# zeroQiaoba/MERTools

Measured on NVIDIA H100. Metric: clips/sec tri-modal feature-extract + fusion-train step, higher is better.
Workload: dtype f16 operands (ViT / HuBERT / BERT layers, ViT attention) / tf32 (audio + text attention, patch embed) / f16 (HuBERT conv1-2) / bf16x3 (HuBERT conv3-6, feature projection) tensor-core products, fp32 accumulate; fp32 elsewhere

## Files before the change

mertools_b200/_lib.py:

```python
from __future__ import annotations

import ctypes as C
import os

_HERE = os.path.dirname(os.path.abspath(__file__))
LIB_PATH = os.path.join(_HERE, "lib", "libmer_b200.so")

MER_EPI_GELU = 1
MER_EPI_ROUND_TF32 = 2
MER_EPI_SPLIT_BF16 = 4
MER_GEMM_TF32 = 0
MER_GEMM_BF16X3 = 1
MER_GEMM_F16 = 2
MER_EPI_OUT_F16 = 16
MER_LN_OUT_F16 = 8
MER_ATT_QKV_F16 = 32
MER_LN_ROUND_TF32 = 1
MER_LN_ACC_INIT = 2
MER_LN_ACC_ADD = 4


class MerError(RuntimeError):
    pass


class MerGemmEpilogue(C.Structure):
    _fields_ = [
        ("bias", C.c_void_p), ("res", C.c_void_p), ("out", C.c_void_p),
        ("out_bstride", C.c_longlong), ("out_row0", C.c_longlong),
        ("res_bstride", C.c_longlong), ("res_row0", C.c_longlong),
        ("ld_out", C.c_int), ("ld_res", C.c_int), ("flags", C.c_int), ("split_off", C.c_int),
        ("vt", C.c_void_p), ("vt_ld", C.c_longlong), ("vt_col0", C.c_int),
    ]


class MerGemmDesc(C.Structure):
    _fields_ = [
        ("A", C.c_void_p), ("W", C.c_void_p),
        ("rows_per_batch", C.c_int), ("a_rows_dim", C.c_int), ("batches", C.c_int),
        ("N", C.c_int), ("K_inner", C.c_int), ("taps", C.c_int), ("P", C.c_int),
        ("a_phase_stride", C.c_longlong), ("a_row_stride", C.c_longlong),
        ("a_batch_stride", C.c_longlong), ("force_block_n", C.c_int), ("mode", C.c_int),
        ("cluster", C.c_int), ("a_row0", C.c_int), ("a_cols", C.c_int), ("a_col_group", C.c_int),
        ("ep", MerGemmEpilogue),
    ]


_lib = None


def lib() -> C.CDLL:
    global _lib
    if _lib is None:
        if not os.path.exists(LIB_PATH):
            raise MerError(
                f"{LIB_PATH} not found: run `python -c 'import __graft_entry__ as g; g.build()'` "
                "(no CPU fallback exists for the mertools_b200 hot path)")
        _lib = C.CDLL(LIB_PATH)
        _lib.mer_last_error.restype = C.c_char_p
        _declare(_lib)
    return _lib


def _declare(l):
    vp, i32, i64, f32 = C.c_void_p, C.c_int, C.c_longlong, C.c_float
    sig = {
        "mer_abi_version": [],
        "mer_check_device": [],
        "mer_gemm": [C.POINTER(MerGemmDesc), vp],
        "mer_layernorm": [vp, vp, vp, vp, vp, vp, i64, i32, f32, i32, vp],
        "mer_round_tf32": [vp, i64, vp],
        "mer_split_bf16": [vp, vp, i64, i32, vp],
        "mer_attention": [vp, vp, i64, vp, vp, i32, i64, i32, i32, i32, vp],
    }
    for name, args in sig.items():
        fn = getattr(l, name)
        fn.argtypes = args
        fn.restype = C.c_int


def declare(name, args):
    fn = getattr(lib(), name)
    fn.argtypes = args
    fn.restype = C.c_int
    return fn


def check(rc: int):
    if rc != 0:
        raise MerError(f"libmer_b200 error {rc}: {lib().mer_last_error().decode(errors='replace')}")


def ptr(t):
    if t is None:
        return None
    return C.c_void_p(t.data_ptr())


def stream_ptr():
    import torch
    return C.c_void_p(torch.cuda.current_stream().cuda_stream)


def gemm(A, W, out, *, bias=None, res=None, gelu=False, round_out=False, split_out=False,
         mode=MER_GEMM_TF32, rows_per_batch=None, batches=1, a_rows_dim=None, K_inner=None, taps=1, P=1,
         a_phase_stride=0, a_row_stride=None, a_batch_stride=0,
         out_bstride=0, out_row0=0, res_bstride=0, res_row0=0,
         ld_out=None, ld_res=None, force_block_n=0, cluster=0, vt=None, vt_col0=0, gelu_libm=False,
         f16_out=False, a_row0=0, a_cols=0, a_col_group=0):
    N, K = W.shape
    d = MerGemmDesc()
    d.A, d.W = A.data_ptr(), W.data_ptr()
    d.taps, d.P = taps, P
    d.K_inner = K_inner if K_inner is not None else K // taps
    assert d.K_inner * taps == K
    d.rows_per_batch = rows_per_batch if rows_per_batch is not None else A.shape[0]
    d.a_rows_dim = a_rows_dim if a_rows_dim is not None else d.rows_per_batch
    d.batches = batches
    d.N = N
    d.a_phase_stride = a_phase_stride if P > 1 else d.K_inner
    d.a_row_stride = a_row_stride if a_row_stride is not None else K
    d.a_batch_stride = a_batch_stride if batches > 1 else d.a_row_stride * d.a_rows_dim
    d.force_block_n = force_block_n
    d.mode = mode
    d.cluster = cluster
    d.a_row0, d.a_cols, d.a_col_group = a_row0, a_cols, a_col_group
    d.ep.bias = bias.data_ptr() if bias is not None else None
    d.ep.res = res.data_ptr() if res is not None else None
    d.ep.out = out.data_ptr()
    d.ep.out_bstride, d.ep.out_row0 = out_bstride, out_row0
    d.ep.res_bstride, d.ep.res_row0 = res_bstride, res_row0
    d.ep.ld_out = ld_out if ld_out is not None else N
    d.ep.ld_res = ld_res if ld_res is not None else N
    d.ep.flags = ((MER_EPI_GELU if gelu else 0) | (MER_EPI_ROUND_TF32 if round_out else 0)
                  | (MER_EPI_SPLIT_BF16 if split_out else 0) | (8 if gelu_libm else 0)
                  | (MER_EPI_OUT_F16 if f16_out else 0))
    d.ep.split_off = N
    if vt is not None:
        d.ep.vt, d.ep.vt_ld, d.ep.vt_col0 = vt.data_ptr(), vt.shape[1], vt_col0
    check(lib().mer_gemm(C.byref(d), stream_ptr()))
    return out


gemm_tf32 = gemm


def layernorm(x, gamma, beta, y, *, eps, y_split=None, acc=None, flags=0):
    rows = x.numel() // x.shape[-1]
    check(lib().mer_layernorm(ptr(x), ptr(gamma), ptr(beta), ptr(y), ptr(y_split), ptr(acc), rows,
                              x.shape[-1], eps, flags, stream_ptr()))
    return y


def split_bf16(x):
    import torch
    x = x.contiguous()
    out = torch.empty_like(x)
    check(lib().mer_split_bf16(ptr(x), ptr(out), x.numel() // x.shape[-1], x.shape[-1], stream_ptr()))
    return out


def unsplit_bf16(xs):
    import torch
    K = xs.shape[-1]
    b = xs.contiguous().view(torch.bfloat16).view(*xs.shape[:-1], K // 32, 2, 32).float()
    return (b[..., 0, :] + b[..., 1, :]).reshape(*xs.shape[:-1], K)


def round_tf32_(x):
    check(lib().mer_round_tf32(ptr(x), x.numel(), stream_ptr()))
    return x


def attention(qkv, ctx, cu_seqlens, max_seqlen, heads, round_out=False, vt=None, f16_out=False, split_out=False):
    import torch
    if qkv.dtype == torch.float16:
        assert vt is not None and vt.dtype == torch.float16
        if ctx.dtype == torch.float16:
            out_fl = MER_EPI_OUT_F16
        else:
            assert ctx.dtype == torch.float32
            out_fl = MER_EPI_SPLIT_BF16 if split_out else (MER_EPI_ROUND_TF32 if round_out else 0)
        check(lib().mer_attention(ptr(qkv), ptr(vt), vt.shape[1], ptr(ctx), ptr(cu_seqlens),
                                  cu_seqlens.numel() - 1, qkv.shape[0], max_seqlen, heads,
                                  out_fl | MER_ATT_QKV_F16, stream_ptr()))
        return ctx
    check(lib().mer_attention(ptr(qkv), ptr(vt), vt.shape[1] if vt is not None else 0, ptr(ctx),
                              ptr(cu_seqlens), cu_seqlens.numel() - 1, qkv.shape[0], max_seqlen, heads,
                              MER_EPI_OUT_F16 if f16_out else (MER_EPI_ROUND_TF32 if round_out else 0),
                              stream_ptr()))
    return ctx
```

mertools_b200/csrc/gemm.cu:

```cuda
#include <stdlib.h>

#include "mer_common.cuh"
#include "mer_kernels.h"

namespace {

using namespace mer;

constexpr int BLOCK_M = 128;
constexpr int BLOCK_K = 32;
constexpr int CONSUMERS = 2;
constexpr int NUM_THREADS = 128 * (1 + CONSUMERS);

template <int BLOCK_N, int MODE>
struct GemmCfg {
  static constexpr bool kSplit = MODE == MER_GEMM_BF16X3;
  static constexpr bool kF16 = MODE == MER_GEMM_F16;
  static constexpr int kBlockK = kF16 ? 64 : BLOCK_K;
  static constexpr int kRowBytes = 128;
  static constexpr int kKind = kSplit ? 1 : (kF16 ? 0 : 2);
  static constexpr int kABytes = BLOCK_M * kRowBytes;
  static constexpr int kBBytes = BLOCK_N * kRowBytes;
  static constexpr int kStageBytes = kABytes + kBBytes;
  static constexpr int kStages = BLOCK_N == 256 ? 4 : 6;
  static constexpr int kBarBytes = 256;
  static constexpr int kSmemBytes = kStages * kStageBytes + kBarBytes + 1024;
  static_assert(kSmemBytes <= 227 * 1024, "shared memory budget");
};

constexpr int EPI_GELU_PACKED = 1 << 16;

template <int GELU>
__device__ __forceinline__ float epi_act(float v) {
  if (GELU == 1) return gelu_erf_fast(v);
  if (GELU == 2) return gelu_erf(v);
  if (GELU == 3) return quick_gelu_fast(v);
  return v;
}
template <int GELU>
__device__ __forceinline__ void epi_act2(float a, float b, float& ga, float& gb) {
  if (GELU == 5) {
    gelu_erf_fast2(a, b, ga, gb);
  } else {
    ga = epi_act<GELU>(a);
    gb = epi_act<GELU>(b);
  }
}

template <int NH, int GELU, int OUT, bool RES>
__device__ __forceinline__ void epi_tile(float (&acc)[NH][64], const MerGemmEpilogue& ep, int n_base, int m_base,
                                         int rows_per_batch, long long out_row_b, long long res_row_b, int wg_row0) {
  constexpr bool kVt = GELU == 0 && !RES;
  const int lane = threadIdx.x & 31, w = (threadIdx.x >> 5) & 3;
  const int g = lane >> 2, t = lane & 3;
#pragma unroll
  for (int i = 0; i < 2; ++i) {
    const int m = m_base + wg_row0 + 16 * w + g + 8 * i;
    if (m >= rows_per_batch) continue;
    const long long orow = out_row_b + m;
    const float* rrow = RES ? ep.res + (res_row_b + m) * (long long)ep.ld_res : nullptr;
#pragma unroll
    for (int hh = 0; hh < NH; ++hh) {
#pragma unroll
      for (int j = 0; j < 16; ++j) {
        const int n = n_base + 128 * hh + 8 * j + 2 * t;
        float v0 = acc[hh][4 * j + 2 * i], v1 = acc[hh][4 * j + 2 * i + 1];
        if (ep.bias) {
          const float2 q = __ldg(reinterpret_cast<const float2*>(ep.bias + n));
          v0 += q.x;
          v1 += q.y;
        }
        if (kVt && ep.vt != nullptr && n >= ep.vt_col0) {
          const long long vo = (long long)(n - ep.vt_col0) * ep.vt_ld + orow;
          if (OUT == 3) {
            uint16_t* vt16 = reinterpret_cast<uint16_t*>(ep.vt) + vo;
            const uint32_t p = pack_f16x2(v0, v1);
            vt16[0] = (uint16_t)(p & 0xffffu);
            vt16[ep.vt_ld] = (uint16_t)(p >> 16);
          } else {
            if (OUT == 1) {
              v0 = round_tf32(v0);
              v1 = round_tf32(v1);
            }
            ep.vt[vo] = v0;
            ep.vt[vo + ep.vt_ld] = v1;
          }
          continue;
        }
        epi_act2<GELU>(v0, v1, v0, v1);
        if (RES) {
          const float2 r = __ldg(reinterpret_cast<const float2*>(rrow + n));
          v0 += r.x;
          v1 += r.y;
        }
        if (GELU == 4) {
          v0 = fmaxf(v0, 0.f);
          v1 = fmaxf(v1, 0.f);
        }
        if (OUT == 3) {
          *reinterpret_cast<uint32_t*>(reinterpret_cast<uint16_t*>(ep.out) + orow * ep.ld_out + n) = pack_f16x2(v0, v1);
        } else if (OUT == 2) {
          store_split2(ep.out + orow * ep.ld_out, n, v0, v1);
        } else {
          if (OUT == 1) {
            v0 = round_tf32(v0);
            v1 = round_tf32(v1);
          }
          *reinterpret_cast<float2*>(ep.out + orow * ep.ld_out + n) = make_float2(v0, v1);
        }
      }
    }
  }
}

template <int BLOCK_N, int MODE>
__global__ void __launch_bounds__(NUM_THREADS, 1)
gemm_kernel(const __grid_constant__ CUtensorMap tmap_a,
            const __grid_constant__ CUtensorMap tmap_b, const MerGemmEpilogue ep,
            int rows_per_batch, int batches, int N, int K, int K_inner, int P, int a_row0, int a_col_group) {
  using Cfg = GemmCfg<BLOCK_N, MODE>;
  constexpr int NH = BLOCK_N / 128;
  extern __shared__ uint8_t smem_raw[];
  uint8_t* smem = smem_raw + ((1024u - (smem_u32(smem_raw) & 1023u)) & 1023u);
  uint8_t* smem_a = smem;
  uint8_t* smem_b = smem + Cfg::kStages * Cfg::kABytes;
  uint64_t* bars = reinterpret_cast<uint64_t*>(smem + Cfg::kStages * Cfg::kStageBytes);
  uint64_t* full_bar = bars;
  uint64_t* empty_bar = bars + Cfg::kStages;

  const int wg = threadIdx.x >> 7;
  const int warp = threadIdx.x >> 5;
  const int lane = threadIdx.x & 31;

  const int m_tiles = (rows_per_batch + BLOCK_M - 1) / BLOCK_M;
  const int n_tiles = N / BLOCK_N;
  const int num_kb = K / Cfg::kBlockK;
  const int num_tiles = batches * m_tiles * n_tiles;

  if (threadIdx.x == 0) {
    tma_prefetch_desc(&tmap_a);
    tma_prefetch_desc(&tmap_b);
    for (int i = 0; i < Cfg::kStages; ++i) {
      mbar_init(&full_bar[i], 1);
      mbar_init(&empty_bar[i], 4 * CONSUMERS);
    }
    fence_mbar_init();
  }
  __syncthreads();

  if (wg == 0) {
    asm volatile("setmaxnreg.dec.sync.aligned.u32 40;\n" ::: "memory");
    if (warp != 0) return;
    int stage = 0;
    uint32_t phase = 0;
    constexpr int kEl = Cfg::kSplit ? 2 : 1;
    for (int t = blockIdx.x; t < num_tiles; t += gridDim.x) {
      const int n_blk = t % n_tiles;
      const int mb = t / n_tiles;
      const int b = mb / m_tiles;
      const int mt = mb % m_tiles;
      int c0 = 0, tap_phase = 0, tap_row = 0;
      const int c_win = a_col_group > 0 ? ((n_blk * BLOCK_N) / a_col_group) * a_col_group : 0;
      const int row_base = mt * BLOCK_M + a_row0;
      for (int kb = 0; kb < num_kb; ++kb) {
        mbar_wait_nocall(&empty_bar[stage], phase ^ 1);
        if (elect_one()) {
          mbar_expect_tx(&full_bar[stage], Cfg::kStageBytes);
          tma_load_4d(smem_a + stage * Cfg::kABytes, &tmap_a, &full_bar[stage], (c_win + c0) * kEl, tap_phase,
                      row_base + tap_row, b);
          tma_load_2d(smem_b + stage * Cfg::kBBytes, &tmap_b, &full_bar[stage], kb * Cfg::kBlockK * kEl,
                      n_blk * BLOCK_N);
        }
        __syncwarp();
        c0 += Cfg::kBlockK;
        if (c0 == K_inner) {
          c0 = 0;
          if (++tap_phase == P) {
            tap_phase = 0;
            ++tap_row;
          }
        }
        if (++stage == Cfg::kStages) {
          stage = 0;
          phase ^= 1;
        }
      }
    }
    return;
  }

  asm volatile("setmaxnreg.inc.sync.aligned.u32 232;\n" ::: "memory");
  const int wg_row0 = (wg - 1) * 64;
  const uint64_t desc_a0 = wgmma_desc_sw128(smem_u32(smem_a + wg_row0 * Cfg::kRowBytes));
  const uint64_t desc_b0 = wgmma_desc_sw128(smem_u32(smem_b));
  const int gelu_kind = (ep.flags & MER_EPI_RELU) ? 4 : (ep.flags & MER_EPI_QUICK_GELU) ? 3
                        : (ep.flags & MER_EPI_GELU)
                            ? ((ep.flags & MER_EPI_GELU_LIBM) ? 2 : ((ep.flags & EPI_GELU_PACKED) ? 5 : 1)) : 0;
  const int out_kind = (ep.flags & MER_EPI_OUT_F16) ? 3 : (ep.flags & MER_EPI_SPLIT_BF16) ? 2 :
                       ((ep.flags & MER_EPI_ROUND_TF32) ? 1 : 0);
  const int kind = gelu_kind * 4 + out_kind;
  int stage = 0;
  uint32_t phase = 0;
  float acc[NH][64];
  for (int t = blockIdx.x; t < num_tiles; t += gridDim.x) {
    const int n_blk = t % n_tiles;
    const int mb = t / n_tiles;
    const int b = mb / m_tiles;
    const int mt = mb % m_tiles;
    int prev_stage = -1;
    for (int kb = 0; kb < num_kb; ++kb) {
      mbar_wait_nocall(&full_bar[stage], phase);
      const uint64_t da = desc_a0 + (uint64_t)(stage * (Cfg::kABytes >> 4));
      const uint64_t db = desc_b0 + (uint64_t)(stage * (Cfg::kBBytes >> 4));
      constexpr uint64_t kHalfB = (128 * Cfg::kRowBytes) >> 4;
      wgmma_fence();
#pragma unroll
      for (int k = 0; k < (Cfg::kSplit ? 2 : 4); ++k) {
#pragma unroll
        for (int hh = 0; hh < NH; ++hh) {
          const uint64_t dbh = db + hh * kHalfB;
          if (!Cfg::kSplit) {
            wgmma_m64n128<Cfg::kKind>(acc[hh], da + 2 * k, dbh + 2 * k, (kb | k) != 0);
          } else {
            wgmma_m64n128<1>(acc[hh], da + 2 * k, dbh + 2 * k, (kb | k) != 0);
            wgmma_m64n128<1>(acc[hh], da + 4 + 2 * k, dbh + 2 * k, 1);
            wgmma_m64n128<1>(acc[hh], da + 2 * k, dbh + 4 + 2 * k, 1);
          }
        }
      }
      wgmma_commit();
      wgmma_wait<1>();
      if (prev_stage >= 0 && lane == 0) mbar_arrive(&empty_bar[prev_stage]);
      prev_stage = stage;
      if (++stage == Cfg::kStages) {
        stage = 0;
        phase ^= 1;
      }
    }
    wgmma_wait<0>();
#pragma unroll
    for (int hh = 0; hh < NH; ++hh)
#pragma unroll
      for (int r = 0; r < 64; ++r) wgmma_fence_operand(acc[hh][r]);
    if (lane == 0) mbar_arrive(&empty_bar[prev_stage]);

    const int n_base = n_blk * BLOCK_N;
    const int m_base = mt * BLOCK_M;
    const long long out_row_b = (long long)b * ep.out_bstride + ep.out_row0;
    const long long res_row_b = (long long)b * ep.res_bstride + ep.res_row0;
#define MER_EPI(G, O, R) epi_tile<NH, G, O, R>(acc, ep, n_base, m_base, rows_per_batch, out_row_b, res_row_b, wg_row0)
    if (ep.res != nullptr) {
      if (gelu_kind == 4) MER_EPI(4, 0, true);
      else if (gelu_kind != 0) MER_EPI(1, 0, true);
      else if (out_kind == 1) MER_EPI(0, 1, true);
      else MER_EPI(0, 0, true);
    } else {
      switch (kind) {
        case 0: MER_EPI(0, 0, false); break;
        case 1: MER_EPI(0, 1, false); break;
        case 2: MER_EPI(0, 2, false); break;
        case 3: MER_EPI(0, 3, false); break;
        case 4: MER_EPI(1, 0, false); break;
        case 5: MER_EPI(1, 1, false); break;
        case 6: MER_EPI(1, 2, false); break;
        case 7: MER_EPI(1, 3, false); break;
        case 8: MER_EPI(2, 0, false); break;
        case 9: MER_EPI(2, 1, false); break;
        case 10: MER_EPI(2, 2, false); break;
        case 11: MER_EPI(2, 3, false); break;
        case 13: MER_EPI(3, 1, false); break;
        case 15: MER_EPI(3, 3, false); break;
        case 16: MER_EPI(4, 0, false); break;
        case 22: MER_EPI(5, 2, false); break;
        case 23: MER_EPI(5, 3, false); break;
        default: MER_EPI(3, 0, false); break;
      }
    }
#undef MER_EPI
  }
}

long long g_variant_launches[8] = {};

template <int BLOCK_N, int MODE>
int launch_gemm(const MerGemmDesc* g, cudaStream_t stream) {
  using Cfg = GemmCfg<BLOCK_N, MODE>;
  ++g_variant_launches[(MODE & 3) | (BLOCK_N == 256 ? 4 : 0)];
  CUtensorMap ta, tb;
  const CUtensorMapDataType dt = Cfg::kSplit ? CU_TENSOR_MAP_DATA_TYPE_BFLOAT16
                                 : Cfg::kF16 ? CU_TENSOR_MAP_DATA_TYPE_FLOAT16
                                             : CU_TENSOR_MAP_DATA_TYPE_FLOAT32;
  const CUtensorMapSwizzle sw = CU_TENSOR_MAP_SWIZZLE_128B;
  const uint64_t mult = Cfg::kSplit ? 2 : 1;
  const uint64_t sbytes = Cfg::kF16 ? 2 : 4;
  {
    const uint64_t dims[4] = {(uint64_t)(g->a_cols > 0 ? g->a_cols : g->K_inner) * mult, (uint64_t)g->P,
                              (uint64_t)g->a_rows_dim, (uint64_t)g->batches};
    const uint64_t strides[3] = {(uint64_t)g->a_phase_stride * sbytes,
                                 (uint64_t)g->a_row_stride * sbytes,
                                 (uint64_t)g->a_batch_stride * sbytes};
    const uint32_t box[4] = {(uint32_t)(Cfg::kBlockK * mult), 1, BLOCK_M, 1};
    if (int rc = mer_make_tmap(&ta, dt, 4, g->A, dims, strides, box, sw)) return rc;
  }
  {
    const int K = g->K_inner * g->taps;
    const uint64_t dims[2] = {(uint64_t)K * mult, (uint64_t)g->N};
    const uint64_t strides[1] = {(uint64_t)K * sbytes};
    const uint32_t box[2] = {(uint32_t)(Cfg::kBlockK * mult), BLOCK_N};
    if (int rc = mer_make_tmap(&tb, dt, 2, g->W, dims, strides, box, sw)) return rc;
  }
  static MerPerDevice attr_set;
  if (attr_set.needs_setup()) {
    MER_CUDA_CHECK(cudaFuncSetAttribute(gemm_kernel<BLOCK_N, MODE>, cudaFuncAttributeMaxDynamicSharedMemorySize,
                                        Cfg::kSmemBytes));
    attr_set.mark();
  }
  const int m_tiles = (g->rows_per_batch + BLOCK_M - 1) / BLOCK_M;
  const long long tiles = (long long)g->batches * m_tiles * (g->N / BLOCK_N);
  MER_REQUIRE(tiles < (1ll << 31), "mer_gemm: %lld tiles", tiles);
  int grid = mer_num_sms();
  if (tiles < grid) grid = (int)tiles;
  const int klass = (MODE == MER_GEMM_F16 && (long long)g->rows_per_batch * g->batches < (1ll << 17)) ? MER_PROF_F16_SMALL
                                                                                                        : MODE;
  const int prof = mer_prof_begin(klass, 2.0 * (double)g->rows_per_batch * g->batches * g->N *
                                             (double)(g->K_inner * g->taps), stream);
  MerGemmEpilogue ep = g->ep;
  {
    const bool plain_gelu = (ep.flags & MER_EPI_GELU) && !(ep.flags & MER_EPI_GELU_LIBM) && !ep.res;
    if (plain_gelu && (ep.flags & (MER_EPI_OUT_F16 | MER_EPI_SPLIT_BF16))) {
      const char* e = getenv("MER_GELU_PACKED");
      if (e && atoi(e) == 1) ep.flags |= EPI_GELU_PACKED;
    }
  }
  gemm_kernel<BLOCK_N, MODE><<<grid, NUM_THREADS, Cfg::kSmemBytes, stream>>>(
      ta, tb, ep, g->rows_per_batch, g->batches, g->N, g->K_inner * g->taps, g->K_inner, g->P, g->a_row0,
      g->a_col_group);
  MER_CUDA_CHECK(cudaGetLastError());
  mer_count_launches(1);
  mer_prof_end(prof, stream);
  return 0;
}

}

extern "C" long long mer_gemm_variant_launches(int block_n, int mode, int cluster, int twosm) {
  if ((block_n != 128 && block_n != 256) || mode < 0 || mode > 2 || cluster < 1 || cluster > 2) return -1;
  if (cluster != 1 || twosm) return 0;
  return g_variant_launches[(mode & 3) | (block_n == 256 ? 4 : 0)];
}

int mer_gemm_launch(const MerGemmDesc* g, cudaStream_t stream) {
  MER_REQUIRE(g && g->A && g->W && g->ep.out, "mer_gemm: null operand");
  MER_REQUIRE(g->mode == MER_GEMM_TF32 || g->mode == MER_GEMM_BF16X3 || g->mode == MER_GEMM_F16,
              "mer_gemm: unknown mode %d", g->mode);
  const int kstep = g->mode == MER_GEMM_F16 ? 64 : BLOCK_K;
  const int salign = g->mode == MER_GEMM_F16 ? 8 : 4;

  MER_REQUIRE(g->K_inner > 0 && g->K_inner % kstep == 0 && g->taps > 0 && g->P > 0,
              "mer_gemm: K_inner=%d must be a positive multiple of %d (taps=%d P=%d)",
              g->K_inner, kstep, g->taps, g->P);
  MER_REQUIRE(g->a_rows_dim >= g->rows_per_batch, "mer_gemm: a_rows_dim < rows_per_batch");
  MER_REQUIRE(g->N > 0 && g->N % 128 == 0, "mer_gemm: N=%d must be a multiple of 128", g->N);
  MER_REQUIRE(g->rows_per_batch > 0 && g->batches > 0, "mer_gemm: empty problem");
  MER_REQUIRE(g->a_row_stride % salign == 0 && g->a_batch_stride % salign == 0 &&
                  g->a_phase_stride % salign == 0,
              "mer_gemm: A strides must be multiples of 16 bytes");
  MER_REQUIRE(!((g->ep.flags & MER_EPI_OUT_F16) &&
                ((g->ep.flags & (MER_EPI_SPLIT_BF16 | MER_EPI_ROUND_TF32)) || g->ep.res)),
              "mer_gemm: an fp16 output excludes the other output formats and a residual");
  MER_REQUIRE(g->ep.ld_out % 4 == 0 && (g->ep.res == nullptr || g->ep.ld_res % 4 == 0),
              "mer_gemm: out/res leading dims must be multiples of 4 floats");
  MER_REQUIRE(!((g->ep.flags & MER_EPI_SPLIT_BF16) && (g->ep.res || g->ep.vt)),
              "mer_gemm: a bf16-split output cannot be combined with a residual or the transposed side output");
  MER_REQUIRE(!(g->ep.res && g->ep.vt), "mer_gemm: a residual cannot be combined with the transposed side output");
  MER_REQUIRE(!(g->ep.res && (g->ep.flags & MER_EPI_GELU) &&
                (g->ep.flags & (MER_EPI_ROUND_TF32 | MER_EPI_GELU_LIBM))),
              "mer_gemm: residual + GELU is available with the polynomial GELU and a plain fp32 output");
  MER_REQUIRE(!((g->ep.flags & MER_EPI_QUICK_GELU) &&
                ((g->ep.flags & (MER_EPI_GELU | MER_EPI_SPLIT_BF16)) || g->ep.res || g->ep.vt)),
              "mer_gemm: quick-GELU comes alone (fp32, tf32 or fp16 output; no residual / split / V^T)");
  MER_REQUIRE(!((g->ep.flags & MER_EPI_RELU) &&
                ((g->ep.flags & (MER_EPI_GELU | MER_EPI_QUICK_GELU | MER_EPI_SPLIT_BF16 | MER_EPI_ROUND_TF32 |
                                 MER_EPI_OUT_F16)) || g->ep.vt)),
              "mer_gemm: ReLU goes with a plain fp32 output (optionally + residual)");
  MER_REQUIRE(g->a_col_group == 0 || g->force_block_n == 128 || g->force_block_n == 256,
              "mer_gemm: a_col_group needs force_block_n (the weights are built for one block width)");
  MER_REQUIRE(!(g->ep.vt && (g->ep.flags & MER_EPI_GELU)), "mer_gemm: GELU + transposed side output is not supported");
  const int m_tiles = (g->rows_per_batch + BLOCK_M - 1) / BLOCK_M;
  const long long tiles256 = (g->N % 256 == 0) ? (long long)g->batches * m_tiles * (g->N / 256) : 0;
  const bool wide = (tiles256 >= mer_num_sms() && g->force_block_n != 128) ||
                    (g->force_block_n == 256 && tiles256 > 0);
  if (g->mode == MER_GEMM_F16)
    return wide ? launch_gemm<256, MER_GEMM_F16>(g, stream) : launch_gemm<128, MER_GEMM_F16>(g, stream);
  if (g->mode == MER_GEMM_BF16X3)
    return wide ? launch_gemm<256, MER_GEMM_BF16X3>(g, stream) : launch_gemm<128, MER_GEMM_BF16X3>(g, stream);
  return wide ? launch_gemm<256, MER_GEMM_TF32>(g, stream) : launch_gemm<128, MER_GEMM_TF32>(g, stream);
}
```

mertools_b200/csrc/mer_common.cuh:

```cuda
#pragma once

#include <cuda.h>
#include <cuda_runtime.h>
#include <stdint.h>
#include <stdio.h>
#include <string.h>

void mer_set_error(const char* fmt, ...);

#define MER_CUDA_CHECK(expr)                                                              \
  do {                                                                                    \
    cudaError_t _e = (expr);                                                              \
    if (_e != cudaSuccess) {                                                              \
      mer_set_error("%s:%d: %s -> %s", __FILE__, __LINE__, #expr, cudaGetErrorString(_e)); \
      return 1;                                                                           \
    }                                                                                     \
  } while (0)

#define MER_REQUIRE(cond, ...)      \
  do {                              \
    if (!(cond)) {                  \
      mer_set_error(__VA_ARGS__);   \
      return 2;                     \
    }                               \
  } while (0)

int mer_make_tmap(CUtensorMap* out, CUtensorMapDataType dtype, int rank, const void* base,
                  const uint64_t* dims, const uint64_t* strides_bytes, const uint32_t* box,
                  CUtensorMapSwizzle swizzle);

int mer_num_sms();
void mer_count_launches(int n);

#ifdef __CUDACC__

#ifndef MER_SPIN_LIMIT
#define MER_SPIN_LIMIT (1u << 27)
#endif

namespace mer {

__device__ __forceinline__ uint32_t smem_u32(const void* p) {
  return static_cast<uint32_t>(__cvta_generic_to_shared(p));
}

__device__ __forceinline__ bool elect_one() {
  uint32_t pred = 0;
  asm volatile(
      "{\n\t"
      ".reg .pred P;\n\t"
      "elect.sync _|P, 0xffffffff;\n\t"
      "selp.b32 %0, 1, 0, P;\n\t"
      "}\n"
      : "=r"(pred));
  return pred != 0;
}

__device__ __forceinline__ void mbar_init(uint64_t* bar, uint32_t count) {
  asm volatile("mbarrier.init.shared::cta.b64 [%0], %1;" ::"r"(smem_u32(bar)), "r"(count));
}
__device__ __forceinline__ void fence_mbar_init() {
  asm volatile("fence.mbarrier_init.release.cluster;" ::: "memory");
}
__device__ __forceinline__ void fence_proxy_async() {
  asm volatile("fence.proxy.async.shared::cta;" ::: "memory");
}
__device__ __forceinline__ void mbar_expect_tx(uint64_t* bar, uint32_t bytes) {
  asm volatile("mbarrier.arrive.expect_tx.shared::cta.b64 _, [%0], %1;" ::"r"(smem_u32(bar)),
               "r"(bytes)
               : "memory");
}
__device__ __forceinline__ void mbar_arrive(uint64_t* bar) {
  asm volatile("mbarrier.arrive.shared::cta.b64 _, [%0];" ::"r"(smem_u32(bar)) : "memory");
}
__device__ __forceinline__ bool mbar_try_wait(uint64_t* bar, uint32_t parity) {
  uint32_t ok;
  asm volatile(
      "{\n\t"
      ".reg .pred P;\n\t"
      "mbarrier.try_wait.parity.shared::cta.b64 P, [%1], %2;\n\t"
      "selp.b32 %0, 1, 0, P;\n\t"
      "}\n"
      : "=r"(ok)
      : "r"(smem_u32(bar)), "r"(parity)
      : "memory");
  return ok != 0;
}
__device__ __forceinline__ bool mbar_test_wait(uint64_t* bar, uint32_t parity) {
  uint32_t ok;
  asm volatile(
      "{\n\t"
      ".reg .pred P;\n\t"
      "mbarrier.test_wait.parity.shared::cta.b64 P, [%1], %2;\n\t"
      "selp.b32 %0, 1, 0, P;\n\t"
      "}\n"
      : "=r"(ok)
      : "r"(smem_u32(bar)), "r"(parity)
      : "memory");
  return ok != 0;
}
__device__ __forceinline__ void mbar_wait(uint64_t* bar, uint32_t parity) {
  uint32_t spins = 0;
  while (!mbar_try_wait(bar, parity)) {
    if (++spins > MER_SPIN_LIMIT) {
      printf("mer: mbarrier wait timed out (block %d thread %d)\n", (int)blockIdx.x,
             (int)threadIdx.x);
      __trap();
    }
  }
}
__device__ __forceinline__ void mbar_wait_nocall(uint64_t* bar, uint32_t parity) {
  uint32_t spins = 0;
  while (!mbar_try_wait(bar, parity)) {
    if (++spins > MER_SPIN_LIMIT) __trap();
  }
}

__device__ __forceinline__ void tma_prefetch_desc(const CUtensorMap* m) {
  asm volatile("prefetch.tensormap [%0];" ::"l"(reinterpret_cast<uint64_t>(m)) : "memory");
}
__device__ __forceinline__ void tma_load_2d(void* smem, const CUtensorMap* m, uint64_t* bar,
                                            int c0, int c1) {
  asm volatile(
      "cp.async.bulk.tensor.2d.shared::cluster.global.mbarrier::complete_tx::bytes"
      " [%0], [%1, {%3, %4}], [%2];" ::"r"(smem_u32(smem)),
      "l"(reinterpret_cast<uint64_t>(m)), "r"(smem_u32(bar)), "r"(c0), "r"(c1)
      : "memory");
}
__device__ __forceinline__ void tma_load_3d(void* smem, const CUtensorMap* m, uint64_t* bar,
                                            int c0, int c1, int c2) {
  asm volatile(
      "cp.async.bulk.tensor.3d.shared::cluster.global.mbarrier::complete_tx::bytes"
      " [%0], [%1, {%3, %4, %5}], [%2];" ::"r"(smem_u32(smem)),
      "l"(reinterpret_cast<uint64_t>(m)), "r"(smem_u32(bar)), "r"(c0), "r"(c1), "r"(c2)
      : "memory");
}

__device__ __forceinline__ void tma_load_4d(void* smem, const CUtensorMap* m, uint64_t* bar,
                                            int c0, int c1, int c2, int c3) {
  asm volatile(
      "cp.async.bulk.tensor.4d.shared::cluster.global.mbarrier::complete_tx::bytes"
      " [%0], [%1, {%3, %4, %5, %6}], [%2];" ::"r"(smem_u32(smem)),
      "l"(reinterpret_cast<uint64_t>(m)), "r"(smem_u32(bar)), "r"(c0), "r"(c1), "r"(c2), "r"(c3)
      : "memory");
}

__device__ __forceinline__ uint64_t wgmma_desc_sw128(uint32_t smem_addr) {
  return static_cast<uint64_t>((smem_addr & 0x3FFFF) >> 4) | (1ull << 16) | (uint64_t(1024 >> 4) << 32) |
         (1ull << 62);
}
__device__ __forceinline__ void wgmma_fence() { asm volatile("wgmma.fence.sync.aligned;" ::: "memory"); }
__device__ __forceinline__ void wgmma_commit() { asm volatile("wgmma.commit_group.sync.aligned;" ::: "memory"); }
template <int N>
__device__ __forceinline__ void wgmma_wait() {
  asm volatile("wgmma.wait_group.sync.aligned %0;" ::"n"(N) : "memory");
}
__device__ __forceinline__ void wgmma_fence_operand(float& r) { asm volatile("" : "+f"(r)::"memory"); }

#define MER_WGMMA_D64                                                                                            \
  "{%0, %1, %2, %3, %4, %5, %6, %7, %8, %9, %10, %11, %12, %13, %14, %15, %16, %17, %18, %19, %20, %21, %22, %23, " \
  "%24, %25, %26, %27, %28, %29, %30, %31, %32, %33, %34, %35, %36, %37, %38, %39, %40, %41, %42, %43, %44, %45, "  \
  "%46, %47, %48, %49, %50, %51, %52, %53, %54, %55, %56, %57, %58, %59, %60, %61, %62, %63}"
#define MER_WGMMA_OUT64(d)                                                                                        \
  "+f"(d[0]), "+f"(d[1]), "+f"(d[2]), "+f"(d[3]), "+f"(d[4]), "+f"(d[5]), "+f"(d[6]), "+f"(d[7]), "+f"(d[8]),      \
      "+f"(d[9]), "+f"(d[10]), "+f"(d[11]), "+f"(d[12]), "+f"(d[13]), "+f"(d[14]), "+f"(d[15]), "+f"(d[16]),       \
      "+f"(d[17]), "+f"(d[18]), "+f"(d[19]), "+f"(d[20]), "+f"(d[21]), "+f"(d[22]), "+f"(d[23]), "+f"(d[24]),      \
      "+f"(d[25]), "+f"(d[26]), "+f"(d[27]), "+f"(d[28]), "+f"(d[29]), "+f"(d[30]), "+f"(d[31]), "+f"(d[32]),      \
      "+f"(d[33]), "+f"(d[34]), "+f"(d[35]), "+f"(d[36]), "+f"(d[37]), "+f"(d[38]), "+f"(d[39]), "+f"(d[40]),      \
      "+f"(d[41]), "+f"(d[42]), "+f"(d[43]), "+f"(d[44]), "+f"(d[45]), "+f"(d[46]), "+f"(d[47]), "+f"(d[48]),      \
      "+f"(d[49]), "+f"(d[50]), "+f"(d[51]), "+f"(d[52]), "+f"(d[53]), "+f"(d[54]), "+f"(d[55]), "+f"(d[56]),      \
      "+f"(d[57]), "+f"(d[58]), "+f"(d[59]), "+f"(d[60]), "+f"(d[61]), "+f"(d[62]), "+f"(d[63])

template <int KIND>
__device__ __forceinline__ void wgmma_m64n128(float (&d)[64], uint64_t desc_a, uint64_t desc_b, int accumulate) {
  if (KIND == 0) {
    asm volatile("{\n.reg .pred p;\nsetp.ne.b32 p, %66, 0;\n"
                 "wgmma.mma_async.sync.aligned.m64n128k16.f32.f16.f16 " MER_WGMMA_D64 ", %64, %65, p, 1, 1, 0, 0;\n}\n"
                 : MER_WGMMA_OUT64(d)
                 : "l"(desc_a), "l"(desc_b), "r"(accumulate));
  } else if (KIND == 1) {
    asm volatile("{\n.reg .pred p;\nsetp.ne.b32 p, %66, 0;\n"
                 "wgmma.mma_async.sync.aligned.m64n128k16.f32.bf16.bf16 " MER_WGMMA_D64 ", %64, %65, p, 1, 1, 0, 0;\n}\n"
                 : MER_WGMMA_OUT64(d)
                 : "l"(desc_a), "l"(desc_b), "r"(accumulate));
  } else {
    asm volatile("{\n.reg .pred p;\nsetp.ne.b32 p, %66, 0;\n"
                 "wgmma.mma_async.sync.aligned.m64n128k8.f32.tf32.tf32 " MER_WGMMA_D64 ", %64, %65, p, 1, 1;\n}\n"
                 : MER_WGMMA_OUT64(d)
                 : "l"(desc_a), "l"(desc_b), "r"(accumulate));
  }
}

__device__ __forceinline__ uint32_t cluster_ctarank() {
  uint32_t r;
  asm volatile("mov.u32 %0, %%cluster_ctarank;" : "=r"(r));
  return r;
}
__device__ __forceinline__ void cluster_sync_all() {
  asm volatile("barrier.cluster.arrive.release.aligned;" ::: "memory");
  asm volatile("barrier.cluster.wait.acquire.aligned;" ::: "memory");
}

__device__ __forceinline__ float round_tf32(float x) {
  uint32_t u;
  asm("cvt.rna.tf32.f32 %0, %1;" : "=r"(u) : "f"(x));
  return __uint_as_float(u);
}
__device__ __forceinline__ uint32_t pack_f16x2(float lo, float hi) {
  uint32_t r;
  asm("cvt.rn.satfinite.f16x2.f32 %0, %1, %2;" : "=r"(r) : "f"(hi), "f"(lo));
  return r;
}

__device__ __forceinline__ uint32_t pack_bf16x2(float a, float b) {
  uint32_t r;
  asm("cvt.rn.bf16x2.f32 %0, %1, %2;" : "=r"(r) : "f"(b), "f"(a));
  return r;
}
__device__ __forceinline__ float bf16_round(float x) {
  return __uint_as_float(pack_bf16x2(x, 0.f) << 16);
}
__device__ __forceinline__ int split_index(int col) { return ((col >> 5) << 6) + (col & 31); }
__device__ __forceinline__ void store_split4(void* row_base, int col, float4 v) {
  const float hx = bf16_round(v.x), hy = bf16_round(v.y), hz = bf16_round(v.z), hw = bf16_round(v.w);
  uint16_t* o = reinterpret_cast<uint16_t*>(row_base) + split_index(col);
  *reinterpret_cast<uint2*>(o) = make_uint2(pack_bf16x2(hx, hy), pack_bf16x2(hz, hw));
  *reinterpret_cast<uint2*>(o + 32) =
      make_uint2(pack_bf16x2(v.x - hx, v.y - hy), pack_bf16x2(v.z - hz, v.w - hw));
}
__device__ __forceinline__ void store_split2(void* row_base, int col, float a, float b) {
  const uint32_t hp = pack_bf16x2(a, b);
  const float ha = __uint_as_float(hp << 16), hb = __uint_as_float(hp & 0xffff0000u);
  uint16_t* o = reinterpret_cast<uint16_t*>(row_base) + split_index(col);
  *reinterpret_cast<uint32_t*>(o) = hp;
  *reinterpret_cast<uint32_t*>(o + 32) = pack_bf16x2(a - ha, b - hb);
}
__device__ __forceinline__ void store_split1(void* row_base, int col, float v) {
  const float h = bf16_round(v);
  uint16_t* o = reinterpret_cast<uint16_t*>(row_base) + split_index(col);
  o[0] = (uint16_t)(__float_as_uint(h) >> 16);
  o[32] = (uint16_t)(pack_bf16x2(v - h, 0.f) & 0xFFFFu);
}

__device__ __forceinline__ float gelu_erf(float x) {
  return 0.5f * x * (1.0f + erff(x * 0.70710678118654752440f));
}
__device__ __forceinline__ float gelu_erf_fast(float x) {
  const float z = fabsf(x) * 0.70710678118654752440f;
  float t, e;
  asm("rcp.approx.ftz.f32 %0, %1;" : "=f"(t) : "f"(fmaf(0.3275911f, z, 1.0f)));
  float p = fmaf(1.061405429f, t, -1.453152027f);
  p = fmaf(p, t, 1.421413741f);
  p = fmaf(p, t, -0.284496736f);
  p = fmaf(p, t, 0.254829592f);
  asm("ex2.approx.ftz.f32 %0, %1;" : "=f"(e) : "f"(-1.4426950408889634f * z * z));
  const float erf_abs = fmaf(-p * t, e, 1.0f);
  const float hx = 0.5f * x;
  return fmaf(fabsf(hx), erf_abs, hx);
}

__device__ __forceinline__ float quick_gelu_fast(float x) {
  float e, r;
  asm("ex2.approx.ftz.f32 %0, %1;" : "=f"(e) : "f"(-1.702f * 1.4426950408889634f * x));
  asm("rcp.approx.ftz.f32 %0, %1;" : "=f"(r) : "f"(1.0f + e));
  return x * r;
}

__device__ __forceinline__ float max3(float a, float b, float c) { return fmaxf(fmaxf(a, b), c); }
__device__ __forceinline__ uint64_t pack2(float lo, float hi) {
  uint64_t r;
  asm("mov.b64 %0, {%1, %2};" : "=l"(r) : "f"(lo), "f"(hi));
  return r;
}
__device__ __forceinline__ void unpack2(uint64_t v, float& lo, float& hi) {
  asm("mov.b64 {%0, %1}, %2;" : "=f"(lo), "=f"(hi) : "l"(v));
}
__device__ __forceinline__ uint64_t fma2(uint64_t a, uint64_t b, uint64_t c) {
  float a0, a1, b0, b1, c0, c1;
  unpack2(a, a0, a1);
  unpack2(b, b0, b1);
  unpack2(c, c0, c1);
  return pack2(__fmaf_rn(a0, b0, c0), __fmaf_rn(a1, b1, c1));
}
__device__ __forceinline__ uint64_t mul2(uint64_t a, uint64_t b) {
  float a0, a1, b0, b1;
  unpack2(a, a0, a1);
  unpack2(b, b0, b1);
  return pack2(__fmul_rn(a0, b0), __fmul_rn(a1, b1));
}
__device__ __forceinline__ uint64_t add2(uint64_t a, uint64_t b) {
  float a0, a1, b0, b1;
  unpack2(a, a0, a1);
  unpack2(b, b0, b1);
  return pack2(__fadd_rn(a0, b0), __fadd_rn(a1, b1));
}
__device__ __forceinline__ void ex2_poly2(uint64_t x2, float& a, float& b) {
  float x0, x1;
  unpack2(x2, x0, x1);
  const uint64_t x = pack2(fmaxf(x0, -126.f), fmaxf(x1, -126.f));
  const auto bc = [](float v) { return pack2(v, v); };
  const uint64_t r = add2(x, bc(12582912.f));
  const uint64_t f = fma2(add2(r, bc(-12582912.f)), bc(-1.f), x);
  uint64_t p = fma2(bc(0.00957401655614376f), f, bc(0.055918190628290176f));
  p = fma2(p, f, bc(0.2402464896440506f));
  p = fma2(p, f, bc(0.6931217312812805f));
  p = fma2(p, f, bc(0.9999992847442627f));
  float p0, p1, r0, r1;
  unpack2(p, p0, p1);
  unpack2(r, r0, r1);
  a = __uint_as_float(__float_as_uint(p0) + (__float_as_uint(r0) << 23));
  b = __uint_as_float(__float_as_uint(p1) + (__float_as_uint(r1) << 23));
}
__device__ __forceinline__ void gelu_erf_fast2(float x0, float x1, float& g0, float& g1) {
  const uint64_t x = pack2(x0, x1), ax = pack2(fabsf(x0), fabsf(x1));
  const auto bc = [](float v) { return pack2(v, v); };
  float d0, d1, t0, t1, a0, a1, e0, e1;
  unpack2(fma2(bc(0.3275911f * 0.70710678118654752440f), ax, bc(1.0f)), d0, d1);
  asm("rcp.approx.ftz.f32 %0, %1;" : "=f"(t0) : "f"(d0));
  asm("rcp.approx.ftz.f32 %0, %1;" : "=f"(t1) : "f"(d1));
  const uint64_t t = pack2(t0, t1);
  uint64_t p = fma2(bc(-1.061405429f), t, bc(1.453152027f));
  p = fma2(p, t, bc(-1.421413741f));
  p = fma2(p, t, bc(0.284496736f));
  p = fma2(p, t, bc(-0.254829592f));
  unpack2(mul2(mul2(x, x), bc(-0.5f * 1.4426950408889634f)), a0, a1);
  asm("ex2.approx.ftz.f32 %0, %1;" : "=f"(e0) : "f"(a0));
  asm("ex2.approx.ftz.f32 %0, %1;" : "=f"(e1) : "f"(a1));
  const uint64_t erf_abs = fma2(mul2(p, t), pack2(e0, e1), bc(1.0f));
  unpack2(fma2(mul2(ax, bc(0.5f)), erf_abs, mul2(x, bc(0.5f))), g0, g1);
}

__device__ __forceinline__ float adam_param(float pi, float grad, float& m, float& v, float lr, float beta1, float beta2,
                                            float eps, float wd, float bc1, float bc2_sqrt) {
  grad = __fmaf_rn(wd, pi, grad);
  m = __fmaf_rn(__fsub_rn(grad, m), __fsub_rn(1.f, beta1), m);
  v = __fmaf_rn(v, beta2, __fmul_rn(__fmul_rn(__fsub_rn(1.f, beta2), grad), grad));
  const float denom = __fadd_rn(__fdiv_rn(__fsqrt_rn(v), bc2_sqrt), eps);
  return __fsub_rn(pi, __fmul_rn(__fdiv_rn(lr, bc1), __fdiv_rn(m, denom)));
}

__device__ __forceinline__ float warp_sum(float v) {
#pragma unroll
  for (int o = 16; o > 0; o >>= 1) v += __shfl_xor_sync(0xffffffffu, v, o);
  return v;
}
__device__ __forceinline__ float warp_max(float v) {
#pragma unroll
  for (int o = 16; o > 0; o >>= 1) v = fmaxf(v, __shfl_xor_sync(0xffffffffu, v, o));
  return v;
}

}
#endif
```

Baseline: 894.5.

## Add ping-pong GEMM schedule with 64-row tiles for mid-size tile counts

Adds a ping-pong warp-specialized schedule where the two consumer warpgroups each own a separate 64-row tile and alternate mainloop and epilogue through named barriers. It is chosen automatically when the cooperative tile count falls between one and one-and-a-half waves of SMs. The aim is to hide the epilogue behind the other warpgroup's MMAs and to cut the wave-quantization tail. In exchange each tile has half the rows, so B traffic per output rises, and the new stage and phase bookkeeping adds correctness risk.

```diff
diff --git a/mertools_b200/_lib.py b/mertools_b200/_lib.py
--- a/mertools_b200/_lib.py
+++ b/mertools_b200/_lib.py
@@ -13,6 +13,8 @@
 MER_GEMM_BF16X3 = 1
 MER_GEMM_F16 = 2
 MER_EPI_OUT_F16 = 16
+MER_EPI_QUICK_GELU = 64
+MER_EPI_RELU = 128
 MER_LN_OUT_F16 = 8
 MER_ATT_QKV_F16 = 32
 MER_LN_ROUND_TF32 = 1
@@ -107,7 +109,7 @@
          a_phase_stride=0, a_row_stride=None, a_batch_stride=0,
          out_bstride=0, out_row0=0, res_bstride=0, res_row0=0,
          ld_out=None, ld_res=None, force_block_n=0, cluster=0, vt=None, vt_col0=0, gelu_libm=False,
-         f16_out=False, a_row0=0, a_cols=0, a_col_group=0):
+         f16_out=False, a_row0=0, a_cols=0, a_col_group=0, extra_flags=0):
     N, K = W.shape
     d = MerGemmDesc()
     d.A, d.W = A.data_ptr(), W.data_ptr()
@@ -134,7 +136,7 @@
     d.ep.ld_res = ld_res if ld_res is not None else N
     d.ep.flags = ((MER_EPI_GELU if gelu else 0) | (MER_EPI_ROUND_TF32 if round_out else 0)
                   | (MER_EPI_SPLIT_BF16 if split_out else 0) | (8 if gelu_libm else 0)
-                  | (MER_EPI_OUT_F16 if f16_out else 0))
+                  | (MER_EPI_OUT_F16 if f16_out else 0) | extra_flags)
     d.ep.split_off = N
     if vt is not None:
         d.ep.vt, d.ep.vt_ld, d.ep.vt_col0 = vt.data_ptr(), vt.shape[1], vt_col0
diff --git a/mertools_b200/csrc/gemm.cu b/mertools_b200/csrc/gemm.cu
--- a/mertools_b200/csrc/gemm.cu
+++ b/mertools_b200/csrc/gemm.cu
@@ -12,19 +12,24 @@
 constexpr int CONSUMERS = 2;
 constexpr int NUM_THREADS = 128 * (1 + CONSUMERS);
 
-template <int BLOCK_N, int MODE>
+constexpr int SCHED_COOP = 0;
+constexpr int SCHED_PINGPONG = 1;
+
+template <int BLOCK_N, int MODE, int SCHED>
 struct GemmCfg {
   static constexpr bool kSplit = MODE == MER_GEMM_BF16X3;
   static constexpr bool kF16 = MODE == MER_GEMM_F16;
+  static constexpr int kTileM = SCHED == SCHED_PINGPONG ? 64 : BLOCK_M;
   static constexpr int kBlockK = kF16 ? 64 : BLOCK_K;
   static constexpr int kRowBytes = 128;
   static constexpr int kKind = kSplit ? 1 : (kF16 ? 0 : 2);
-  static constexpr int kABytes = BLOCK_M * kRowBytes;
+  static constexpr int kABytes = kTileM * kRowBytes;
   static constexpr int kBBytes = BLOCK_N * kRowBytes;
   static constexpr int kStageBytes = kABytes + kBBytes;
-  static constexpr int kStages = BLOCK_N == 256 ? 4 : 6;
+  static constexpr int kStages = SCHED == SCHED_PINGPONG ? (BLOCK_N == 256 ? 5 : 8) : (BLOCK_N == 256 ? 4 : 6);
   static constexpr int kBarBytes = 256;
   static constexpr int kSmemBytes = kStages * kStageBytes + kBarBytes + 1024;
+  static_assert(2 * kStages * 8 <= kBarBytes, "barrier area");
   static_assert(kSmemBytes <= 227 * 1024, "shared memory budget");
 };
 
@@ -113,13 +118,96 @@
   }
 }
 
-template <int BLOCK_N, int MODE>
+template <class Cfg, int NH>
+__device__ __forceinline__ int mma_mainloop(float (&acc)[NH][64], uint64_t* full_bar, uint64_t* empty_bar, int& stage,
+                                            uint32_t& phase, int num_kb, uint64_t desc_a0, uint64_t desc_b0,
+                                            int lane) {
+  int prev_stage = -1;
+  for (int kb = 0; kb < num_kb; ++kb) {
+    mbar_wait_nocall(&full_bar[stage], phase);
+    const uint64_t da = desc_a0 + (uint64_t)(stage * (Cfg::kABytes >> 4));
+    const uint64_t db = desc_b0 + (uint64_t)(stage * (Cfg::kBBytes >> 4));
+    constexpr uint64_t kHalfB = (128 * Cfg::kRowBytes) >> 4;
+    wgmma_fence();
+#pragma unroll
+    for (int k = 0; k < (Cfg::kSplit ? 2 : 4); ++k) {
+#pragma unroll
+      for (int hh = 0; hh < NH; ++hh) {
+        const uint64_t dbh = db + hh * kHalfB;
+        if (!Cfg::kSplit) {
+          wgmma_m64n128<Cfg::kKind>(acc[hh], da + 2 * k, dbh + 2 * k, (kb | k) != 0);
+        } else {
+          wgmma_m64n128<1>(acc[hh], da + 2 * k, dbh + 2 * k, (kb | k) != 0);
+          wgmma_m64n128<1>(acc[hh], da + 4 + 2 * k, dbh + 2 * k, 1);
+          wgmma_m64n128<1>(acc[hh], da + 2 * k, dbh + 4 + 2 * k, 1);
+        }
+      }
+    }
+    wgmma_commit();
+    wgmma_wait<1>();
+    if (prev_stage >= 0 && lane == 0) mbar_arrive(&empty_bar[prev_stage]);
+    prev_stage = stage;
+    if (++stage == Cfg::kStages) {
+      stage = 0;
+      phase ^= 1;
+    }
+  }
+  return prev_stage;
+}
+
+template <int NH>
+__device__ __forceinline__ void mma_drain(float (&acc)[NH][64], uint64_t* empty_bar, int last_stage, int lane) {
+  wgmma_wait<0>();
+#pragma unroll
+  for (int hh = 0; hh < NH; ++hh)
+#pragma unroll
+    for (int r = 0; r < 64; ++r) wgmma_fence_operand(acc[hh][r]);
+  if (lane == 0) mbar_arrive(&empty_bar[last_stage]);
+}
+
+template <int NH>
+__device__ __forceinline__ void epilogue(float (&acc)[NH][64], const MerGemmEpilogue& ep, int gelu_kind, int out_kind,
+                                         int n_base, int m_base, int rows_per_batch, long long out_row_b,
+                                         long long res_row_b, int wg_row0) {
+#define MER_EPI(G, O, R) epi_tile<NH, G, O, R>(acc, ep, n_base, m_base, rows_per_batch, out_row_b, res_row_b, wg_row0)
+  if (ep.res != nullptr) {
+    if (gelu_kind == 4) MER_EPI(4, 0, true);
+    else if (gelu_kind != 0) MER_EPI(1, 0, true);
+    else if (out_kind == 1) MER_EPI(0, 1, true);
+    else MER_EPI(0, 0, true);
+  } else {
+    switch (gelu_kind * 4 + out_kind) {
+      case 0: MER_EPI(0, 0, false); break;
+      case 1: MER_EPI(0, 1, false); break;
+      case 2: MER_EPI(0, 2, false); break;
+      case 3: MER_EPI(0, 3, false); break;
+      case 4: MER_EPI(1, 0, false); break;
+      case 5: MER_EPI(1, 1, false); break;
+      case 6: MER_EPI(1, 2, false); break;
+      case 7: MER_EPI(1, 3, false); break;
+      case 8: MER_EPI(2, 0, false); break;
+      case 9: MER_EPI(2, 1, false); break;
+      case 10: MER_EPI(2, 2, false); break;
+      case 11: MER_EPI(2, 3, false); break;
+      case 13: MER_EPI(3, 1, false); break;
+      case 15: MER_EPI(3, 3, false); break;
+      case 16: MER_EPI(4, 0, false); break;
+      case 22: MER_EPI(5, 2, false); break;
+      case 23: MER_EPI(5, 3, false); break;
+      default: MER_EPI(3, 0, false); break;
+    }
+  }
+#undef MER_EPI
+}
+
+template <int BLOCK_N, int MODE, int SCHED>
 __global__ void __launch_bounds__(NUM_THREADS, 1)
 gemm_kernel(const __grid_constant__ CUtensorMap tmap_a,
             const __grid_constant__ CUtensorMap tmap_b, const MerGemmEpilogue ep,
             int rows_per_batch, int batches, int N, int K, int K_inner, int P, int a_row0, int a_col_group) {
-  using Cfg = GemmCfg<BLOCK_N, MODE>;
+  using Cfg = GemmCfg<BLOCK_N, MODE, SCHED>;
   constexpr int NH = BLOCK_N / 128;
+  constexpr bool kPingPong = SCHED == SCHED_PINGPONG;
   extern __shared__ uint8_t smem_raw[];
   uint8_t* smem = smem_raw + ((1024u - (smem_u32(smem_raw) & 1023u)) & 1023u);
   uint8_t* smem_a = smem;
@@ -132,7 +220,7 @@
   const int warp = threadIdx.x >> 5;
   const int lane = threadIdx.x & 31;
 
-  const int m_tiles = (rows_per_batch + BLOCK_M - 1) / BLOCK_M;
+  const int m_tiles = (rows_per_batch + Cfg::kTileM - 1) / Cfg::kTileM;
   const int n_tiles = N / BLOCK_N;
   const int num_kb = K / Cfg::kBlockK;
   const int num_tiles = batches * m_tiles * n_tiles;
@@ -142,7 +230,7 @@
     tma_prefetch_desc(&tmap_b);
     for (int i = 0; i < Cfg::kStages; ++i) {
       mbar_init(&full_bar[i], 1);
-      mbar_init(&empty_bar[i], 4 * CONSUMERS);
+      mbar_init(&empty_bar[i], kPingPong ? 4 : 4 * CONSUMERS);
     }
     fence_mbar_init();
   }
@@ -161,7 +249,7 @@
       const int mt = mb % m_tiles;
       int c0 = 0, tap_phase = 0, tap_row = 0;
       const int c_win = a_col_group > 0 ? ((n_blk * BLOCK_N) / a_col_group) * a_col_group : 0;
-      const int row_base = mt * BLOCK_M + a_row0;
+      const int row_base = mt * Cfg::kTileM + a_row0;
       for (int kb = 0; kb < num_kb; ++kb) {
         mbar_wait_nocall(&empty_bar[stage], phase ^ 1);
         if (elect_one()) {
@@ -190,101 +278,64 @@
   }
 
   asm volatile("setmaxnreg.inc.sync.aligned.u32 232;\n" ::: "memory");
-  const int wg_row0 = (wg - 1) * 64;
-  const uint64_t desc_a0 = wgmma_desc_sw128(smem_u32(smem_a + wg_row0 * Cfg::kRowBytes));
   const uint64_t desc_b0 = wgmma_desc_sw128(smem_u32(smem_b));
   const int gelu_kind = (ep.flags & MER_EPI_RELU) ? 4 : (ep.flags & MER_EPI_QUICK_GELU) ? 3
                         : (ep.flags & MER_EPI_GELU)
                             ? ((ep.flags & MER_EPI_GELU_LIBM) ? 2 : ((ep.flags & EPI_GELU_PACKED) ? 5 : 1)) : 0;
   const int out_kind = (ep.flags & MER_EPI_OUT_F16) ? 3 : (ep.flags & MER_EPI_SPLIT_BF16) ? 2 :
                        ((ep.flags & MER_EPI_ROUND_TF32) ? 1 : 0);
-  const int kind = gelu_kind * 4 + out_kind;
   int stage = 0;
   uint32_t phase = 0;
   float acc[NH][64];
-  for (int t = blockIdx.x; t < num_tiles; t += gridDim.x) {
-    const int n_blk = t % n_tiles;
-    const int mb = t / n_tiles;
-    const int b = mb / m_tiles;
-    const int mt = mb % m_tiles;
-    int prev_stage = -1;
-    for (int kb = 0; kb < num_kb; ++kb) {
-      mbar_wait_nocall(&full_bar[stage], phase);
-      const uint64_t da = desc_a0 + (uint64_t)(stage * (Cfg::kABytes >> 4));
-      const uint64_t db = desc_b0 + (uint64_t)(stage * (Cfg::kBBytes >> 4));
-      constexpr uint64_t kHalfB = (128 * Cfg::kRowBytes) >> 4;
-      wgmma_fence();
-#pragma unroll
-      for (int k = 0; k < (Cfg::kSplit ? 2 : 4); ++k) {
-#pragma unroll
-        for (int hh = 0; hh < NH; ++hh) {
-          const uint64_t dbh = db + hh * kHalfB;
-          if (!Cfg::kSplit) {
-            wgmma_m64n128<Cfg::kKind>(acc[hh], da + 2 * k, dbh + 2 * k, (kb | k) != 0);
-          } else {
-            wgmma_m64n128<1>(acc[hh], da + 2 * k, dbh + 2 * k, (kb | k) != 0);
-            wgmma_m64n128<1>(acc[hh], da + 4 + 2 * k, dbh + 2 * k, 1);
-            wgmma_m64n128<1>(acc[hh], da + 2 * k, dbh + 4 + 2 * k, 1);
-          }
-        }
+  if constexpr (!kPingPong) {
+    const int wg_row0 = (wg - 1) * 64;
+    const uint64_t desc_a0 = wgmma_desc_sw128(smem_u32(smem_a + wg_row0 * Cfg::kRowBytes));
+    for (int t = blockIdx.x; t < num_tiles; t += gridDim.x) {
+      const int n_blk = t % n_tiles;
+      const int mb = t / n_tiles;
+      const int b = mb / m_tiles;
+      const int mt = mb % m_tiles;
+      const int last = mma_mainloop<Cfg>(acc, full_bar, empty_bar, stage, phase, num_kb, desc_a0, desc_b0, lane);
+      mma_drain(acc, empty_bar, last, lane);
+      epilogue(acc, ep, gelu_kind, out_kind, n_blk * BLOCK_N, mt * Cfg::kTileM, rows_per_batch,
+               (long long)b * ep.out_bstride + ep.out_row0, (long long)b * ep.res_bstride + ep.res_row0, wg_row0);
+    }
+  } else {
+    const int c = wg - 1;
+    const uint64_t desc_a0 = wgmma_desc_sw128(smem_u32(smem_a));
+    auto skip_tile = [&]() {
+      const int s = stage + num_kb;
+      stage = s % Cfg::kStages;
+      phase ^= (uint32_t)(s / Cfg::kStages) & 1u;
+    };
+    if (c == 1) skip_tile();
+    for (int t = blockIdx.x + c * gridDim.x; t < num_tiles; t += 2 * gridDim.x) {
+      const int n_blk = t % n_tiles;
+      const int mb = t / n_tiles;
+      const int b = mb / m_tiles;
+      const int mt = mb % m_tiles;
+      if (t >= (int)gridDim.x) {
+        if (c == 0) named_bar_sync<1, 2 * 128>();
+        else named_bar_sync<2, 2 * 128>();
       }
-      wgmma_commit();
-      wgmma_wait<1>();
-      if (prev_stage >= 0 && lane == 0) mbar_arrive(&empty_bar[prev_stage]);
-      prev_stage = stage;
-      if (++stage == Cfg::kStages) {
-        stage = 0;
-        phase ^= 1;
+      const int last = mma_mainloop<Cfg>(acc, full_bar, empty_bar, stage, phase, num_kb, desc_a0, desc_b0, lane);
+      if (t + (int)gridDim.x < num_tiles) {
+        if (c == 0) named_bar_arrive<2, 2 * 128>();
+        else named_bar_arrive<1, 2 * 128>();
       }
-    }
-    wgmma_wait<0>();
-#pragma unroll
-    for (int hh = 0; hh < NH; ++hh)
-#pragma unroll
-      for (int r = 0; r < 64; ++r) wgmma_fence_operand(acc[hh][r]);
-    if (lane == 0) mbar_arrive(&empty_bar[prev_stage]);
-
-    const int n_base = n_blk * BLOCK_N;
-    const int m_base = mt * BLOCK_M;
-    const long long out_row_b = (long long)b * ep.out_bstride + ep.out_row0;
-    const long long res_row_b = (long long)b * ep.res_bstride + ep.res_row0;
-#define MER_EPI(G, O, R) epi_tile<NH, G, O, R>(acc, ep, n_base, m_base, rows_per_batch, out_row_b, res_row_b, wg_row0)
-    if (ep.res != nullptr) {
-      if (gelu_kind == 4) MER_EPI(4, 0, true);
-      else if (gelu_kind != 0) MER_EPI(1, 0, true);
-      else if (out_kind == 1) MER_EPI(0, 1, true);
-      else MER_EPI(0, 0, true);
-    } else {
-      switch (kind) {
-        case 0: MER_EPI(0, 0, false); break;
-        case 1: MER_EPI(0, 1, false); break;
-        case 2: MER_EPI(0, 2, false); break;
-        case 3: MER_EPI(0, 3, false); break;
-        case 4: MER_EPI(1, 0, false); break;
-        case 5: MER_EPI(1, 1, false); break;
-        case 6: MER_EPI(1, 2, false); break;
-        case 7: MER_EPI(1, 3, false); break;
-        case 8: MER_EPI(2, 0, false); break;
-        case 9: MER_EPI(2, 1, false); break;
-        case 10: MER_EPI(2, 2, false); break;
-        case 11: MER_EPI(2, 3, false); break;
-        case 13: MER_EPI(3, 1, false); break;
-        case 15: MER_EPI(3, 3, false); break;
-        case 16: MER_EPI(4, 0, false); break;
-        case 22: MER_EPI(5, 2, false); break;
-        case 23: MER_EPI(5, 3, false); break;
-        default: MER_EPI(3, 0, false); break;
-      }
-    }
-#undef MER_EPI
+      mma_drain(acc, empty_bar, last, lane);
+      epilogue(acc, ep, gelu_kind, out_kind, n_blk * BLOCK_N, mt * Cfg::kTileM, rows_per_batch,
+               (long long)b * ep.out_bstride + ep.out_row0, (long long)b * ep.res_bstride + ep.res_row0, 0);
+      skip_tile();
+    }
   }
 }
 
 long long g_variant_launches[8] = {};
 
-template <int BLOCK_N, int MODE>
+template <int BLOCK_N, int MODE, int SCHED>
 int launch_gemm(const MerGemmDesc* g, cudaStream_t stream) {
-  using Cfg = GemmCfg<BLOCK_N, MODE>;
+  using Cfg = GemmCfg<BLOCK_N, MODE, SCHED>;
   ++g_variant_launches[(MODE & 3) | (BLOCK_N == 256 ? 4 : 0)];
   CUtensorMap ta, tb;
   const CUtensorMapDataType dt = Cfg::kSplit ? CU_TENSOR_MAP_DATA_TYPE_BFLOAT16
@@ -299,7 +350,7 @@
     const uint64_t strides[3] = {(uint64_t)g->a_phase_stride * sbytes,
                                  (uint64_t)g->a_row_stride * sbytes,
                                  (uint64_t)g->a_batch_stride * sbytes};
-    const uint32_t box[4] = {(uint32_t)(Cfg::kBlockK * mult), 1, BLOCK_M, 1};
+    const uint32_t box[4] = {(uint32_t)(Cfg::kBlockK * mult), 1, (uint32_t)Cfg::kTileM, 1};
     if (int rc = mer_make_tmap(&ta, dt, 4, g->A, dims, strides, box, sw)) return rc;
   }
   {
@@ -311,11 +362,11 @@
   }
   static MerPerDevice attr_set;
   if (attr_set.needs_setup()) {
-    MER_CUDA_CHECK(cudaFuncSetAttribute(gemm_kernel<BLOCK_N, MODE>, cudaFuncAttributeMaxDynamicSharedMemorySize,
-                                        Cfg::kSmemBytes));
+    MER_CUDA_CHECK(cudaFuncSetAttribute(gemm_kernel<BLOCK_N, MODE, SCHED>,
+                                        cudaFuncAttributeMaxDynamicSharedMemorySize, Cfg::kSmemBytes));
     attr_set.mark();
   }
-  const int m_tiles = (g->rows_per_batch + BLOCK_M - 1) / BLOCK_M;
+  const int m_tiles = (g->rows_per_batch + Cfg::kTileM - 1) / Cfg::kTileM;
   const long long tiles = (long long)g->batches * m_tiles * (g->N / BLOCK_N);
   MER_REQUIRE(tiles < (1ll << 31), "mer_gemm: %lld tiles", tiles);
   int grid = mer_num_sms();
@@ -332,13 +383,18 @@
       if (e && atoi(e) == 1) ep.flags |= EPI_GELU_PACKED;
     }
   }
-  gemm_kernel<BLOCK_N, MODE><<<grid, NUM_THREADS, Cfg::kSmemBytes, stream>>>(
+  gemm_kernel<BLOCK_N, MODE, SCHED><<<grid, NUM_THREADS, Cfg::kSmemBytes, stream>>>(
       ta, tb, ep, g->rows_per_batch, g->batches, g->N, g->K_inner * g->taps, g->K_inner, g->P, g->a_row0,
       g->a_col_group);
   MER_CUDA_CHECK(cudaGetLastError());
   mer_count_launches(1);
   mer_prof_end(prof, stream);
   return 0;
+}
+
+template <int BLOCK_N, int MODE>
+int launch_sched(const MerGemmDesc* g, cudaStream_t stream, bool coop) {
+  return coop ? launch_gemm<BLOCK_N, MODE, SCHED_COOP>(g, stream) : launch_gemm<BLOCK_N, MODE, SCHED_PINGPONG>(g, stream);
 }
 
 }
@@ -390,9 +446,14 @@
   const long long tiles256 = (g->N % 256 == 0) ? (long long)g->batches * m_tiles * (g->N / 256) : 0;
   const bool wide = (tiles256 >= mer_num_sms() && g->force_block_n != 128) ||
                     (g->force_block_n == 256 && tiles256 > 0);
+  const long long tiles_coop = wide ? tiles256 : (long long)g->batches * m_tiles * (g->N / 128);
+  const long long sms = mer_num_sms();
+  const char* e = getenv("MER_GEMM_COOP");
+  const bool coop = e && *e ? atoi(e) == 1 : !(tiles_coop > sms && 2 * tiles_coop <= 3 * sms);
   if (g->mode == MER_GEMM_F16)
-    return wide ? launch_gemm<256, MER_GEMM_F16>(g, stream) : launch_gemm<128, MER_GEMM_F16>(g, stream);
+    return wide ? launch_sched<256, MER_GEMM_F16>(g, stream, coop) : launch_sched<128, MER_GEMM_F16>(g, stream, coop);
   if (g->mode == MER_GEMM_BF16X3)
-    return wide ? launch_gemm<256, MER_GEMM_BF16X3>(g, stream) : launch_gemm<128, MER_GEMM_BF16X3>(g, stream);
-  return wide ? launch_gemm<256, MER_GEMM_TF32>(g, stream) : launch_gemm<128, MER_GEMM_TF32>(g, stream);
-}
+    return wide ? launch_sched<256, MER_GEMM_BF16X3>(g, stream, coop)
+                : launch_sched<128, MER_GEMM_BF16X3>(g, stream, coop);
+  return wide ? launch_sched<256, MER_GEMM_TF32>(g, stream, coop) : launch_sched<128, MER_GEMM_TF32>(g, stream, coop);
+}
diff --git a/mertools_b200/csrc/mer_common.cuh b/mertools_b200/csrc/mer_common.cuh
--- a/mertools_b200/csrc/mer_common.cuh
+++ b/mertools_b200/csrc/mer_common.cuh
@@ -114,6 +114,15 @@
   while (!mbar_try_wait(bar, parity)) {
     if (++spins > MER_SPIN_LIMIT) __trap();
   }
+}
+
+template <int ID, int THREADS>
+__device__ __forceinline__ void named_bar_sync() {
+  asm volatile("bar.sync %0, %1;" ::"n"(ID), "n"(THREADS) : "memory");
+}
+template <int ID, int THREADS>
+__device__ __forceinline__ void named_bar_arrive() {
+  asm volatile("bar.arrive %0, %1;" ::"n"(ID), "n"(THREADS) : "memory");
 }
 
 __device__ __forceinline__ void tma_prefetch_desc(const CUtensorMap* m) {
```

After: 894.7, median of 6. About the same (+0.0%).
